# DJjjjhao/FIRA-ICSE

Measured on AMD Instinct MI355X. Metric: training commits/sec (FIRA default config), higher is better.
Workload: dtype f32; 1 GPU; BASELINE configs[1]: FIRA training step (fwd+bwd+Adam, dropout 0.1/0.2), batch 32 commits/GPU, fp32, 650-node graphs (mean nnz 1066/graph), vocab 24650; global_batch=32, parallelism=dp1

## Files before the change

### fira_icse_amd/_lib.py

```python
from __future__ import annotations

import ctypes as C
import os

HERE = os.path.dirname(os.path.abspath(__file__))
LIB_PATH = os.environ.get("FIRA_HIP_LIB") or os.path.join(HERE, "libfira_hip.so")


class FiraError(RuntimeError):
    pass


class Dims(C.Structure):
    _fields_ = [("sou_len", C.c_int32), ("sub_len", C.c_int32), ("ast_len", C.c_int32), ("tar_len", C.c_int32),
                ("d_model", C.c_int32), ("n_head", C.c_int32), ("n_layer", C.c_int32), ("vocab", C.c_int32),
                ("ast_vocab", C.c_int32), ("d_ff", C.c_int32)]


class Batch(C.Structure):
    _fields_ = [("B", C.c_int32), ("nnz", C.c_int32), ("sou", C.c_void_p), ("tar", C.c_void_p), ("mark", C.c_void_p),
                ("ast_change", C.c_void_p), ("tar_label", C.c_void_p), ("sub_token", C.c_void_p),
                ("n_nodes", C.c_int32), ("node_rows", C.c_void_p), ("rowptr", C.c_void_p), ("col", C.c_void_p),
                ("val", C.c_void_p), ("n_code", C.c_int32), ("code_rows", C.c_void_p), ("code_mark", C.c_void_p),
                ("n_mem", C.c_int32), ("mem_rows", C.c_void_p), ("mem_dst", C.c_void_p), ("head_rows", C.c_void_p),
# ... 36 lines not shown
    "fira_abi_version": (_I, []),
    "fira_param_count": (_I, [_DP]),
    "fira_param_info": (_I, [_DP, _I, C.c_char_p, C.POINTER(_L), C.POINTER(_L), C.POINTER(C.c_int32), C.POINTER(_L)]),
    "fira_param_total": (_L, [_DP]),
    "fira_workspace_bytes": (_Z, [_DP, _I, _I]),
    "fira_decode_workspace_bytes": (_Z, [_DP, _I, _I]),
    "fira_decode_workspace_bytes_ex": (_Z, [_DP, _I, _I, _I]),
    "fira_gemm_f32": (_I, [_P, _I, _I, _I, _I, _I, _P, _I, _P, _I, _P, _I, _P, _I, _I]),
    "fira_gemm_bf16": (_I, [_P, _I, _I, _I, _I, _I, _P, _I, _P, _I, _P, _I, _P, _I, _I]),
    "fira_weight_shadow": (_I, [_P, _I, _I, _P, _P, _P]),
    "fira_gemm_bf16_wb": (_I, [_P, _I, _I, _I, _P, _I, _P, _I, _P, _I, _P, _I, _I]),
    "fira_csr_spmm_f32": (_I, [_P, _I, _P, _P, _P, _P, _I, _P, _I, _I, _I]),
    "fira_csr_spmm": (_I, [_P, _I, _L, _P, _P, _P, _P, _I, _P, _I, _I, _I, _I]),
    "fira_gcn_layer_fwd": (_I, [_P, _I, _P, _P, _P, _P, _P, _P, _P, _P, _P, _P, _P, _P, _P, _F, _U64, _U32, _I]),
    "fira_gcn_layer_bwd": (_I, [_P, _I, _P, _P, _P, _P, _P, _P, _P, _I]),
    "fira_gcn_weight_planes": (_I, [_P, _I, _P, _P]),
    "fira_linear_x3": (_I, [_P, _I, _I, _P, _I, _P, _P, _P, _I, _I]),
    "fira_linear_dgrad_x3": (_I, [_P, _I, _I, _P, _I, _P, _P, _I, _I, _I]),
    "fira_dgrad_x3_splitk_planes_bytes": (_Z, [_I]),
    "fira_dgrad_x3_splitk": (_I, [_P, _I, _I, _P, _I, _P, _P, _P, _I, _I]),
    "fira_head_logits_x3_scratch_bytes": (_Z, [_I]),
    "fira_head_logits_x3": (_I, [_P, _I, _I, _P, _I, _P, _P, _P, _I, _P]),
    "fira_combination_block_fwd": (_I, [_P, _I, _P, _P, _P, _P, _P, _P, _P, _I, _P, _P, _P, _P, _P, _P, _P, _P, _P, _F, _U64, _U32, _U32, _I]),
    "fira_combination_block_bwd": (_I, [_P, _I, _P, _P, _P, _P, _P, _P, _P, _P, _P, _I, _P, _P, _P, _P, _P, _P, _I, _P, _F, _U64, _U32, _U32, _I]),
    "fira_combination_block_bwd_part_floats": (_I, []),
    "fira_embed_gather_fwd": (_I, [_P, _I, _I, _P, _P, _P, _P, _I, _I]),
    "fira_embed_gather_bwd": (_I, [_P, _I, _I, _P, _P, _P, _I, _I, _I]),
    "fira_combination_fwd": (_I, [_P, _I, _P, _P, _P, _P, _F, _U64, _U32]),
    "fira_combination_bwd": (_I, [_P, _I, _P, _P, _P, _P, _P, _P, _F, _U64, _U32]),
    "fira_add_layernorm_fwd": (_I, [_P, _I, _P, _P, _P, _P, _P, _P, _F, _U64, _U32]),
    "fira_linear_presum_f32": (_I, [_P, _I, _I, _P, _I, _P, _P, _P, _P, _F, _U64, _U32]),
    "fira_ln_linear_f32": (_I, [_P, _I, _I, _P, _I, _P, _P, _P, _I, _I, _P, _P, _P, _P]),
    "fira_ln_bwd_linear_f32": (_I, [_P, _I, _I, _P, _P, _P, _P, _P, _P, _P, _P, _P, _P, _P, _P, _F, _U64, _U32]),
    "fira_linear_layernorm_bf16_fwd": (_I, [_P, _I, _P, _I, _P, _I, _P, _P, _P, _P, _P, _P, _P, _F, _U64, _U32]),
    "fira_add_layernorm_bwd": (_I, [_P, _I, _P, _P, _P, _P, _P, _P, _P, _P, _F, _U64, _U32]),
    "fira_dropout_mask": (_I, [_P, _U64, _U32, _L, _F, _P]),
    "fira_colsum_f32": (_I, [_P, _I, _I, _P, _I, _P]),
    "fira_attention_fwd": (_I, [_P, _I, _I, _I, _I, _P, _I, _P, _I, _P, _I, _P, _I, _I, _P, _I]),
    "fira_attention_bwd": (_I, [_P, _I, _I, _I, _I, _P, _I, _P, _I, _P, _I, _P, _I, _I, _P, _I, _P, _I,
                                _P, _I, _P, _I, _P, _I]),
    "fira_attention_fwd_ex": (_I, [_P, _I, _I, _I, _I, _P, _I, _P, _I, _P, _I, _P, _I, _I, _P, _I, _P, _I, _I, _P]),
    "fira_attention_bwd_ex": (_I, [_P, _I, _I, _I, _I, _P, _I, _P, _I, _P, _I, _P, _I, _I, _P, _I, _P, _I,
                                   _P, _I, _P, _I, _P, _I, _P, _I, _I, _P]),
    "fira_decode_attention": (_I, [_P, _I, _I, _I, _P, _I, _P, _I, _P, _I, _P, _P, _I, _I, _I, _I, _P, _P, _I, _P, _P, _P]),
    "fira_copy_score_fwd": (_I, [_P, _I, _I, _I, _P, _P, _P, _P, _P]),
    "fira_copy_score_bwd": (_I, [_P, _I, _I, _I, _P, _P, _P, _P, _P, _P, _P, _P]),
    "fira_head_loss": (_I, [_P, _I, _I, _I, _I, _P, _P, _I, _P, _P, _P, _P, _P, _P, _P, _I]),
    "fira_adam_step": (_I, [_P, _L, _P, _P, _P, _P, _F, _F, _F, _F, _I, _P]),
    "fira_adam_step_mb": (_I, [_P, _L, _P, _P, _P, _P, _P, _F, _F, _F, _F, _I, _P, _P]),
    "fira_inv_count": (_I, [_P, _P, _P]),
    "fira_adam_step_count": (_I, [_P, _L, _P, _P, _P, _P, _F, _F, _F, _F, _I, _P]),
    "fira_pack_stats": (_I, [_P, _P, _P, _P]),
    "fira_debug_chain": (_I, [_P, _I, _I, _P]),
    "fira_train_fwd_bwd": (_I, [_P, _DP, _BP, _P, _P, _P, _Z, _OP, _P, _P, _P]),
    "fira_train_step": (_I, [_P, _DP, _BP, _P, _P, _P, _Z, _OP, _P, _P, C.POINTER(AdamOpts)]),
    "fira_gemm_wgrad_panel": (_I, [_P, _I, _I, _I, _I, _P, _I, _P, _I, _P, _I, _P, _P, _Z]),
    "fira_ffn_fwd": (_I, [_P, _I, _I] + [_P] * 11 + [_F, _U64, _U32, _I]),
    "fira_ffn_bwd": (_I, [_P, _I, _I] + [_P] * 17 + [_F, _U64, _U32, _I]),
    "fira_head_topk": (_I, [_P, _I, _I, _I, _P, _P, _P, _P, _I, _P, _P, _I]),
    "fira_train_step_rows": (_I, [_P, _DP, _BP, _P, _P, _P, _Z, _OP, _P, _P, C.POINTER(AdamOpts), _P]),
    "fira_adam_rows_sync": (_I, [_P, _DP, _P, C.POINTER(AdamOpts), _P]),
    "fira_adam_rows_catchup": (_I, [_P, _DP, _P, C.POINTER(AdamOpts), _P, _I, _P, _I]),
    "fira_adam_rows_step": (_I, [_P, _DP, _P, _P, C.POINTER(AdamOpts), _P, _P, _P, _I]),
    "fira_train_step_begin_rows": (_I, [_P, _DP, _BP, _P, _P, _P, _Z, _OP, _P, _P, _P, C.POINTER(AdamOpts), _P]),
    "fira_train_step_end_rows": (_I, [_P, _P, C.POINTER(AdamOpts), _P, _P, _P]),
    "fira_ema_update": (_I, [_P, _L, _P, _P, _F]),
# ... 120 lines not shown
```

### fira_icse_amd/csrc/gemm_small.hip

```cpp
#include "engine.h"
#include "epilogue.h"
#include <stdlib.h>

namespace fira {

typedef float f32x16 __attribute__((ext_vector_type(16)));
typedef float f32x4 __attribute__((ext_vector_type(4)));

template <bool B_KCONTIG>
__global__ __launch_bounds__(256) void gemm_small_kernel(int M, int N, int K, const float* __restrict__ A, int lda,
                                                         const float* __restrict__ B, int ldb, float* __restrict__ C,
                                                         int ldc, const float* __restrict__ bias, int flags,
                                                         const int32_t* __restrict__ c_rows,
                                                         const float* __restrict__ relu_mask) {
    __shared__ float red[4][1024];
    const int lane = threadIdx.x & 63, wave = threadIdx.x >> 6;
    const int l31 = lane & 31, kh = lane >> 5;
    const int m0 = blockIdx.y * 32, n0 = blockIdx.x * 32;
    const float* pa = A + (size_t)min(m0 + l31, M - 1) * lda + kh * 16;
    const float* pb = B_KCONTIG ? B + (size_t)min(n0 + l31, N - 1) * ldb + kh * 16
                                : B + (size_t)(kh * 16) * ldb + min(n0 + l31, N - 1);
    f32x16 acc;
#pragma unroll
    for (int r = 0; r < 16; ++r) acc[r] = 0.f;
// ... 105 lines not shown
        const char* pb = slot + 4096 + fb;
        f32x4 vb0, vb1, vb2, vb3;
        vb0.x = *reinterpret_cast<const float*>(pb);        vb0.y = *reinterpret_cast<const float*>(pb + 128);
        vb0.z = *reinterpret_cast<const float*>(pb + 256);  vb0.w = *reinterpret_cast<const float*>(pb + 384);
        vb1.x = *reinterpret_cast<const float*>(pb + 512);  vb1.y = *reinterpret_cast<const float*>(pb + 640);
        vb1.z = *reinterpret_cast<const float*>(pb + 768);  vb1.w = *reinterpret_cast<const float*>(pb + 896);
        vb2.x = *reinterpret_cast<const float*>(pb + 1024); vb2.y = *reinterpret_cast<const float*>(pb + 1152);
        vb2.z = *reinterpret_cast<const float*>(pb + 1280); vb2.w = *reinterpret_cast<const float*>(pb + 1408);
        vb3.x = *reinterpret_cast<const float*>(pb + 1536); vb3.y = *reinterpret_cast<const float*>(pb + 1664);
        vb3.z = *reinterpret_cast<const float*>(pb + 1792); vb3.w = *reinterpret_cast<const float*>(pb + 1920);
        FIRA_MFMA4(va0, vb0) FIRA_MFMA4(va1, vb1) FIRA_MFMA4(va2, vb2) FIRA_MFMA4(va3, vb3)
    }
    return acc;
}

struct LnA {
    const float* gamma = nullptr;
    const float* beta = nullptr;
    float* x_out = nullptr;
    float* stats_out = nullptr;
};

struct LnB {
    const float* sum = nullptr;
    const float* stats = nullptr;
    const float* gamma = nullptr;
    float* ds = nullptr;
    float* dx = nullptr;
    float* part = nullptr;
    float p = 0.f, inv_keep = 1.f;
    uint64_t seed = 0;
    uint32_t site = 0;
    uint32_t idx0 = 0;
};

template <bool B_KCONTIG, int NCH, bool LN_A = false, bool LN_B = false, int NW = 4>
__global__ __launch_bounds__(NW * 64) void gemm_tile32_kernel(int M, int N, const float* __restrict__ A, int lda,
                                                          const float* __restrict__ B, int ldb, float* __restrict__ C,
                                                          int ldc, const float* __restrict__ bias, int flags,
                                                          const int32_t* __restrict__ c_rows,
                                                          const float* __restrict__ relu_mask,
                                                          const int32_t* __restrict__ a_rows, int tiles_n, const EpiRes er,
                                                          const LnA ln, const LnB lb) {
    static_assert(NW == 4 || (!LN_A && !LN_B), "the LayerNorm prologues are written for four waves");
    extern __shared__ __attribute__((aligned(16))) char tile32_dyn[];
    __shared__ __attribute__((aligned(16))) char smem4[NW == 4 ? 4 * 8192 : 16];
    char* const smem = NW == 4 ? smem4 : tile32_dyn;
    __shared__ float ln_red[2][4][32];
    const int lane = threadIdx.x & 63;
    const int wave = __builtin_amdgcn_readfirstlane(threadIdx.x >> 6);
    int t;
    {
        const int b = blockIdx.x, nwg = gridDim.x, q = nwg >> 3, r = nwg & 7, x = b & 7;
        t = (x < r ? x * (q + 1) : r * (q + 1) + (x - r) * q) + (b >> 3);
    }
    const int m0 = (t / tiles_n) * 32, n0 = (t % tiles_n) * 32;
    char* slot = smem + wave * 8192;
    const int lr = lane >> 3, ls = lane & 7;
    const int sw_even = lr >> 1, sw_odd = 4 + (lr >> 1);
    int ra0 = min(m0 + lr, M - 1), ra1 = min(m0 + 8 + lr, M - 1), ra2 = min(m0 + 16 + lr, M - 1), ra3 = min(m0 + 24 + lr, M - 1);
    if (a_rows) { ra0 = a_rows[ra0]; ra1 = a_rows[ra1]; ra2 = a_rows[ra2]; ra3 = a_rows[ra3]; }
    const float* pa0 = A + (size_t)ra0 * lda + ((ls ^ sw_even) << 2);
    const float* pa1 = A + (size_t)ra1 * lda + ((ls ^ sw_odd) << 2);
    const float* pa2 = A + (size_t)ra2 * lda + ((ls ^ sw_even) << 2);
    const float* pa3 = A + (size_t)ra3 * lda + ((ls ^ sw_odd) << 2);
    const float *pb0, *pb1, *pb2, *pb3;
    if (B_KCONTIG) {
        pb0 = B + (size_t)min(n0 + lr, N - 1) * ldb + ((ls ^ sw_even) << 2);
        pb1 = B + (size_t)min(n0 + 8 + lr, N - 1) * ldb + ((ls ^ sw_odd) << 2);
        pb2 = B + (size_t)min(n0 + 16 + lr, N - 1) * ldb + ((ls ^ sw_even) << 2);
        pb3 = B + (size_t)min(n0 + 24 + lr, N - 1) * ldb + ((ls ^ sw_odd) << 2);
    } else {
        pb0 = B + (size_t)lr * ldb + n0 + (ls << 2);
        pb1 = pb0 + (size_t)8 * ldb;
        pb2 = pb0 + (size_t)16 * ldb;
        pb3 = pb0 + (size_t)24 * ldb;
    }
    const int i31 = lane & 31, kh = lane >> 5;
    const int wr_off = lr * 128 + ls * 16;
    const int sw_i = swz8(i31);
    const int fa0 = i31 * 128 + (((kh * 4 + 0) ^ sw_i) << 4), fa1 = i31 * 128 + (((kh * 4 + 1) ^ sw_i) << 4);
    const int fa2 = i31 * 128 + (((kh * 4 + 2) ^ sw_i) << 4), fa3 = i31 * 128 + (((kh * 4 + 3) ^ sw_i) << 4);
    const int fb = kh * 16 * 128 + i31 * 4;
    f32x16 acc;
#pragma unroll
    for (int r = 0; r < 16; ++r) acc[r] = 0.f;
    ChunkRegs R0, R1;
    tile32_fetch<B_KCONTIG>(R0, pa0, pa1, pa2, pa3, pb0, pb1, pb2, pb3, wave << 5, ldb);
    if (NCH > 1) tile32_fetch<B_KCONTIG>(R1, pa0, pa1, pa2, pa3, pb0, pb1, pb2, pb3, (wave + NW) << 5, ldb);
// ... 49 lines not shown
                if (r3 < M) { ln.stats_out[2 * r3] = mean[3]; ln.stats_out[2 * r3 + 1] = rstd[3]; }
            }
        }
    }
    if constexpr (LN_B) {
        static_assert(!LN_B || (NCH == 2 && !LN_A), "the LayerNorm-backward prologue needs the whole row in the two chunks of the four waves");
        auto hsum = [](const f32x4 v) { return (v.x + v.y) + (v.z + v.w); };
        const int ce = (ls ^ sw_even) << 2, co = (ls ^ sw_odd) << 2;
        const int k0 = wave << 5, k1 = (wave + 4) << 5;
        const float* ps0 = lb.sum + (size_t)ra0 * FIRA_D; const float* ps1 = lb.sum + (size_t)ra1 * FIRA_D;
        const float* ps2 = lb.sum + (size_t)ra2 * FIRA_D; const float* ps3 = lb.sum + (size_t)ra3 * FIRA_D;
        f32x4 s00 = *reinterpret_cast<const f32x4*>(ps0 + k0 + ce), s10 = *reinterpret_cast<const f32x4*>(ps0 + k1 + ce);
        f32x4 s01 = *reinterpret_cast<const f32x4*>(ps1 + k0 + co), s11 = *reinterpret_cast<const f32x4*>(ps1 + k1 + co);
        f32x4 s02 = *reinterpret_cast<const f32x4*>(ps2 + k0 + ce), s12 = *reinterpret_cast<const f32x4*>(ps2 + k1 + ce);
        f32x4 s03 = *reinterpret_cast<const f32x4*>(ps3 + k0 + co), s13 = *reinterpret_cast<const f32x4*>(ps3 + k1 + co);
        const float mean0 = lb.stats[2 * ra0], rstd0 = lb.stats[2 * ra0 + 1], mean1 = lb.stats[2 * ra1], rstd1 = lb.stats[2 * ra1 + 1];
        const float mean2 = lb.stats[2 * ra2], rstd2 = lb.stats[2 * ra2 + 1], mean3 = lb.stats[2 * ra3], rstd3 = lb.stats[2 * ra3 + 1];
        const f32x4 g0e = *reinterpret_cast<const f32x4*>(lb.gamma + k0 + ce), g0o = *reinterpret_cast<const f32x4*>(lb.gamma + k0 + co);
        const f32x4 g1e = *reinterpret_cast<const f32x4*>(lb.gamma + k1 + ce), g1o = *reinterpret_cast<const f32x4*>(lb.gamma + k1 + co);
        s00 = (s00 - mean0) * rstd0; s10 = (s10 - mean0) * rstd0; s01 = (s01 - mean1) * rstd1; s11 = (s11 - mean1) * rstd1;
        s02 = (s02 - mean2) * rstd2; s12 = (s12 - mean2) * rstd2; s03 = (s03 - mean3) * rstd3; s13 = (s13 - mean3) * rstd3;
        const f32x4 h00 = R0.a0 * g0e, h10 = R1.a0 * g1e, h01 = R0.a1 * g0o, h11 = R1.a1 * g1o;
        const f32x4 h02 = R0.a2 * g0e, h12 = R1.a2 * g1e, h03 = R0.a3 * g0o, h13 = R1.a3 * g1o;
        {
            const float p0 = sum8(hsum(h00) + hsum(h10)), p1 = sum8(hsum(h01) + hsum(h11));
            const float p2 = sum8(hsum(h02) + hsum(h12)), p3 = sum8(hsum(h03) + hsum(h13));
            const float q0 = sum8(hsum(h00 * s00) + hsum(h10 * s10)), q1 = sum8(hsum(h01 * s01) + hsum(h11 * s11));
            const float q2 = sum8(hsum(h02 * s02) + hsum(h12 * s12)), q3 = sum8(hsum(h03 * s03) + hsum(h13 * s13));
            if (ls == 0) {
                ln_red[0][wave][lr] = p0; ln_red[0][wave][8 + lr] = p1; ln_red[0][wave][16 + lr] = p2; ln_red[0][wave][24 + lr] = p3;
                ln_red[1][wave][lr] = q0; ln_red[1][wave][8 + lr] = q1; ln_red[1][wave][16 + lr] = q2; ln_red[1][wave][24 + lr] = q3;
            }
        }
        if (lb.part && n0 == 0) {
            const bool v0 = m0 + lr < M, v1 = m0 + 8 + lr < M, v2 = m0 + 16 + lr < M, v3 = m0 + 24 + lr < M;
            const f32x4 z = {0.f, 0.f, 0.f, 0.f};
            const f32x4 d00 = v0 ? R0.a0 : z, d10 = v0 ? R1.a0 : z, d01 = v1 ? R0.a1 : z, d11 = v1 ? R1.a1 : z;
            const f32x4 d02 = v2 ? R0.a2 : z, d12 = v2 ? R1.a2 : z, d03 = v3 ? R0.a3 : z, d13 = v3 ? R1.a3 : z;
            float* sc = reinterpret_cast<float*>(slot);
            float colsum[2];
#pragma unroll
            for (int pass = 0; pass < 2; ++pass) {
                __builtin_amdgcn_wave_barrier();
                *reinterpret_cast<f32x4*>(sc + (lr) * 64 + ce) = pass ? d00 : d00 * s00;
                *reinterpret_cast<f32x4*>(sc + (lr) * 64 + 32 + ce) = pass ? d10 : d10 * s10;
                *reinterpret_cast<f32x4*>(sc + (8 + lr) * 64 + co) = pass ? d01 : d01 * s01;
                *reinterpret_cast<f32x4*>(sc + (8 + lr) * 64 + 32 + co) = pass ? d11 : d11 * s11;
                *reinterpret_cast<f32x4*>(sc + (16 + lr) * 64 + ce) = pass ? d02 : d02 * s02;
                *reinterpret_cast<f32x4*>(sc + (16 + lr) * 64 + 32 + ce) = pass ? d12 : d12 * s12;
                *reinterpret_cast<f32x4*>(sc + (24 + lr) * 64 + co) = pass ? d03 : d03 * s03;
                *reinterpret_cast<f32x4*>(sc + (24 + lr) * 64 + 32 + co) = pass ? d13 : d13 * s13;
                __builtin_amdgcn_fence(__ATOMIC_RELEASE, "wavefront");
                __builtin_amdgcn_wave_barrier();
                __builtin_amdgcn_fence(__ATOMIC_ACQUIRE, "wavefront");
                float a0 = 0.f, a1 = 0.f;
#pragma unroll
                for (int r = 0; r < 32; r += 2) { a0 += sc[r * 64 + lane]; a1 += sc[(r + 1) * 64 + lane]; }
                colsum[pass] = a0 + a1;
            }
            const int col = ((wave + 4 * (lane >> 5)) << 5) + (lane & 31);
            float* pp = lb.part + (size_t)(m0 >> 5) * (2 * FIRA_D);
            pp[col] = colsum[0];
            pp[FIRA_D + col] = colsum[1];
        }
        __syncthreads();
        float m1[4], m2[4];
#pragma unroll
        for (int j = 0; j < 4; ++j) {
            m1[j] = ((ln_red[0][0][8 * j + lr] + ln_red[0][1][8 * j + lr]) + (ln_red[0][2][8 * j + lr] + ln_red[0][3][8 * j + lr])) * (1.0f / FIRA_D);
            m2[j] = ((ln_red[1][0][8 * j + lr] + ln_red[1][1][8 * j + lr]) + (ln_red[1][2][8 * j + lr] + ln_red[1][3][8 * j + lr])) * (1.0f / FIRA_D);
        }
        const f32x4 e00 = (h00 - m1[0] - s00 * m2[0]) * rstd0, e10 = (h10 - m1[0] - s10 * m2[0]) * rstd0;
        const f32x4 e01 = (h01 - m1[1] - s01 * m2[1]) * rstd1, e11 = (h11 - m1[1] - s11 * m2[1]) * rstd1;
        const f32x4 e02 = (h02 - m1[2] - s02 * m2[2]) * rstd2, e12 = (h12 - m1[2] - s12 * m2[2]) * rstd2;
        const f32x4 e03 = (h03 - m1[3] - s03 * m2[3]) * rstd3, e13 = (h13 - m1[3] - s13 * m2[3]) * rstd3;
        auto drop = [&](const f32x4 v, int row, int col) {
            if (lb.p <= 0.f) return v;
            const uint32_t e0 = lb.idx0 + (uint32_t)row * FIRA_D + (uint32_t)col;
            return f32x4{v.x * dropout_scale(lb.seed, lb.site, e0, lb.p, lb.inv_keep), v.y * dropout_scale(lb.seed, lb.site, e0 + 1, lb.p, lb.inv_keep),
                         v.z * dropout_scale(lb.seed, lb.site, e0 + 2, lb.p, lb.inv_keep), v.w * dropout_scale(lb.seed, lb.site, e0 + 3, lb.p, lb.inv_keep)};
        };
        const int r0 = m0 + lr, r1 = m0 + 8 + lr, r2 = m0 + 16 + lr, r3 = m0 + 24 + lr;
        R0.a0 = drop(e00, r0, k0 + ce); R1.a0 = drop(e10, r0, k1 + ce); R0.a1 = drop(e01, r1, k0 + co); R1.a1 = drop(e11, r1, k1 + co);
        R0.a2 = drop(e02, r2, k0 + ce); R1.a2 = drop(e12, r2, k1 + ce); R0.a3 = drop(e03, r3, k0 + co); R1.a3 = drop(e13, r3, k1 + co);
        if (n0 == 0) {
            float* o1 = lb.ds;
            float* o2 = lb.dx;
            if (r0 < M) { *reinterpret_cast<f32x4*>(o1 + (size_t)r0 * FIRA_D + k0 + ce) = e00; *reinterpret_cast<f32x4*>(o1 + (size_t)r0 * FIRA_D + k1 + ce) = e10;
                          *reinterpret_cast<f32x4*>(o2 + (size_t)r0 * FIRA_D + k0 + ce) = R0.a0; *reinterpret_cast<f32x4*>(o2 + (size_t)r0 * FIRA_D + k1 + ce) = R1.a0; }
            if (r1 < M) { *reinterpret_cast<f32x4*>(o1 + (size_t)r1 * FIRA_D + k0 + co) = e01; *reinterpret_cast<f32x4*>(o1 + (size_t)r1 * FIRA_D + k1 + co) = e11;
                          *reinterpret_cast<f32x4*>(o2 + (size_t)r1 * FIRA_D + k0 + co) = R0.a1; *reinterpret_cast<f32x4*>(o2 + (size_t)r1 * FIRA_D + k1 + co) = R1.a1; }
            if (r2 < M) { *reinterpret_cast<f32x4*>(o1 + (size_t)r2 * FIRA_D + k0 + ce) = e02; *reinterpret_cast<f32x4*>(o1 + (size_t)r2 * FIRA_D + k1 + ce) = e12;
                          *reinterpret_cast<f32x4*>(o2 + (size_t)r2 * FIRA_D + k0 + ce) = R0.a2; *reinterpret_cast<f32x4*>(o2 + (size_t)r2 * FIRA_D + k1 + ce) = R1.a2; }
            if (r3 < M) { *reinterpret_cast<f32x4*>(o1 + (size_t)r3 * FIRA_D + k0 + co) = e03; *reinterpret_cast<f32x4*>(o1 + (size_t)r3 * FIRA_D + k1 + co) = e13;
                          *reinterpret_cast<f32x4*>(o2 + (size_t)r3 * FIRA_D + k0 + co) = R0.a3; *reinterpret_cast<f32x4*>(o2 + (size_t)r3 * FIRA_D + k1 + co) = R1.a3; }
        }
    }
#pragma unroll
    for (int ci = 0; ci < NCH; ++ci) {
        if ((ci & 1) == 0) {
            tile32_stage(R0, slot, wr_off);
            if (ci + 2 < NCH) tile32_fetch<B_KCONTIG>(R0, pa0, pa1, pa2, pa3, pb0, pb1, pb2, pb3, (wave + NW * (ci + 2)) << 5, ldb);
        } else {
            tile32_stage(R1, slot, wr_off);
            if (ci + 2 < NCH) tile32_fetch<B_KCONTIG>(R1, pa0, pa1, pa2, pa3, pb0, pb1, pb2, pb3, (wave + NW * (ci + 2)) << 5, ldb);
        }
        acc = tile32_compute<B_KCONTIG>(slot, fa0, fa1, fa2, fa3, fb, acc);
    }
    __builtin_amdgcn_wave_barrier();
    float* red = reinterpret_cast<float*>(slot);
#pragma unroll
    for (int r = 0; r < 16; ++r) red[r * 64 + lane] = acc[r];
    __syncthreads();
    {
        constexpr int NV = (16 + NW - 1) / NW;
        const int lnn = threadIdx.x & 63;
        float vals[NV];
        int rows[NV];
        const float* p0 = reinterpret_cast<const float*>(smem);
#pragma unroll
        for (int i = 0; i < NV; ++i) {
            const int idx = threadIdx.x + NW * 64 * i, r = idx >> 6;
            const bool in = (16 % NW == 0) || idx < 1024;
            const int ix = in ? idx : threadIdx.x;
            if constexpr (NW == 4) {
                vals[i] = (p0[ix] + p0[2048 + ix]) + (p0[4096 + ix] + p0[6144 + ix]);
            } else {
                float v = 0.f;
#pragma unroll
                for (int w = 0; w < NW; w += 4)
// ... 72 lines not shown
            *rc = tile32_launch_wide(s, nw, K, tB, grid, M, N, A, lda, B, ldb, C, ldc, bias, flags, c_rows, relu_mask, a_rows, tiles_n, er);
            return true;
        }
    }
#define FIRA_T32(NCH)                                                                                                  \
    case NCH:                                                                                                          \
        if (tB) tile32_launch<true, NCH>(s, grid, M, N, A, lda, B, ldb, C, ldc, bias, flags, c_rows, relu_mask, a_rows, tiles_n, er); \
        else tile32_launch<false, NCH>(s, grid, M, N, A, lda, B, ldb, C, ldc, bias, flags, c_rows, relu_mask, a_rows, tiles_n, er); \
        break;
    switch (nch) { FIRA_T32(1) FIRA_T32(2) FIRA_T32(3) FIRA_T32(4) FIRA_T32(6) FIRA_T32(8) }
#undef FIRA_T32
    hipError_t e = hipGetLastError();
    *rc = e != hipSuccess ? set_err("gemm_tile32: %s", hipGetErrorString(e)) : 0;
    return true;
}

bool gemm_tile32_ln_try(hipStream_t s, int M, int N, const float* S, int lds, const float* W, const float* bias, float* Y,
                        int ldy, int flags, const float* gamma, const float* beta, float* x_out, float* stats_out, int* rc) {
    if (!gemm_tile32_takes(1, M, N, FIRA_D, S, lds, W, FIRA_D)) return false;
    if (((uintptr_t)gamma % 16) || ((uintptr_t)beta % 16) || ((uintptr_t)x_out % 16)) return false;
    ProfScope prof(s, PROF_GEMM, 2.0 * M * N * (double)FIRA_D, 4.0 * ((double)M * FIRA_D + (double)N * FIRA_D + (double)M * N));
    const int tiles_n = cdiv(N, 32);
    LnA ln;
    ln.gamma = gamma; ln.beta = beta; ln.x_out = x_out; ln.stats_out = stats_out;
    hipLaunchKernelGGL((gemm_tile32_kernel<true, 2, true, false>), dim3(cdiv(M, 32) * tiles_n), dim3(256), 0, s, M, N, S, lds, W, FIRA_D,
                       Y, ldy, bias, flags & 3, (const int32_t*)nullptr, (const float*)nullptr, (const int32_t*)nullptr, tiles_n,
                       EpiRes(), ln, LnB());
    hipError_t e = hipGetLastError();
    *rc = e != hipSuccess ? set_err("gemm_tile32_ln: %s", hipGetErrorString(e)) : 0;
    return true;
}

int gemm_tile32_lnb_blocks(int M) { return cdiv(M, 32); }
bool gemm_tile32_lnb_try(hipStream_t s, int M, int N, const float* dy, const float* W, int ldw, float* dX, int lddx,
                         const float* relu_mask, const float* sum, const float* stats, const float* gamma, float* ds,
                         float* dx_drop, float* part, float dropout, uint64_t seed, uint32_t site, int* rc, uint32_t idx0) {
    if (!gemm_tile32_takes(0, M, N, FIRA_D, dy, FIRA_D, W, ldw)) return false;
    if (((uintptr_t)sum % 16) || ((uintptr_t)gamma % 16) || ((uintptr_t)ds % 16) || ((uintptr_t)dx_drop % 16) || ds == dy) return false;
    ProfScope prof(s, PROF_GEMM, 2.0 * M * N * (double)FIRA_D, 4.0 * ((double)M * FIRA_D + (double)N * FIRA_D + (double)M * N));
    const int tiles_n = cdiv(N, 32);
    LnB lb;
    lb.sum = sum; lb.stats = stats; lb.gamma = gamma; lb.ds = ds; lb.dx = dx_drop; lb.part = part;
    lb.p = dropout; lb.inv_keep = dropout > 0.f ? 1.0f / (1.0f - dropout) : 1.0f; lb.seed = seed; lb.site = site; lb.idx0 = idx0;
    hipLaunchKernelGGL((gemm_tile32_kernel<false, 2, false, true>), dim3(cdiv(M, 32) * tiles_n), dim3(256), 0, s, M, N, dy, FIRA_D, W, ldw,
                       dX, lddx, (const float*)nullptr, 0, (const int32_t*)nullptr, relu_mask, (const int32_t*)nullptr, tiles_n,
                       EpiRes(), LnA(), lb);
    hipError_t e = hipGetLastError();
    *rc = e != hipSuccess ? set_err("gemm_tile32_lnb: %s", hipGetErrorString(e)) : 0;
    return true;
}

struct UnfoldGemm { const float *A, *B; float* C; int a_rs, a_ks, b_rs, b_ks, mode; };
struct UnfoldGemmTable { int n = 0; UnfoldGemm e[32]; };
__global__ __launch_bounds__(256) void unfold_gemm_kernel(const UnfoldGemmTable tab) {
    __shared__ float red[4][1024];
    const UnfoldGemm& q = tab.e[blockIdx.y];
    const int lane = threadIdx.x & 63, wave = threadIdx.x >> 6;
    const int l31 = lane & 31, kh = lane >> 5;
    if (q.mode == 2) {
        if (blockIdx.x >= 8) return;
        const f32x4 x = *reinterpret_cast<const f32x4*>(q.B + lane * 4);
        f32x4 a[8];
#pragma unroll
        for (int r = 0; r < 8; ++r)
            a[r] = *reinterpret_cast<const f32x4*>(q.A + (size_t)(blockIdx.x * 32 + wave * 8 + r) * q.a_rs + lane * 4);
#pragma unroll
        for (int r = 0; r < 8; ++r) {
            const float d = wave_sum((a[r].x * x.x + a[r].y * x.y) + (a[r].z * x.z + a[r].w * x.w));
            if (lane == 0) q.C[blockIdx.x * 32 + wave * 8 + r] = d;
        }
        return;
    }
    const int m0 = (blockIdx.x >> 3) * 32, n0 = (blockIdx.x & 7) * 32;
    const float* pa = q.A + (size_t)(m0 + l31) * q.a_rs;
    const float* pb = q.B + (size_t)(n0 + l31) * q.b_rs;
    f32x16 acc;
#pragma unroll
    for (int r = 0; r < 16; ++r) acc[r] = 0.f;
// ... 80 lines not shown
    constexpr long max_tiles = 1024;
    const long tiles = (long)cdiv(M, 32) * cdiv(N, 32);
    if (tA || (M > 64 && tiles > max_tiles) || K % 32 != 0 || K < 64 || lda % 4 != 0 || ((uintptr_t)A % 16) != 0) return false;
    if (tB && (ldb % 4 != 0 || ((uintptr_t)B % 16) != 0)) return false;
    if (gemm_tile32_try(s, tB, M, N, K, A, lda, B, ldb, C, ldc, bias, flags, rc, c_rows, relu_mask, nullptr, nullptr))
        return true;
    dim3 grid(cdiv(N, 32), cdiv(M, 32));
    if (tB) hipLaunchKernelGGL(gemm_small_kernel<true>, grid, dim3(256), 0, s, M, N, K, A, lda, B, ldb, C, ldc, bias, flags, c_rows, relu_mask);
    else hipLaunchKernelGGL(gemm_small_kernel<false>, grid, dim3(256), 0, s, M, N, K, A, lda, B, ldb, C, ldc, bias, flags, c_rows, relu_mask);
    hipError_t e = hipGetLastError();
    if (e != hipSuccess) *rc = set_err("gemm_small: %s", hipGetErrorString(e));
    return true;
}

}

extern "C" {
int fira_linear_presum_f32(void* stream, int M, int K, const float* X, int ldx, const float* W, const float* bias,
                           const float* res, float* sum, float dropout, uint64_t seed, uint32_t stream_id) {
    FIRA_REQUIRE(X && W && res && sum && M > 0, "fira_linear_presum_f32: bad argument");
    FIRA_REQUIRE(dropout >= 0.f && dropout < 1.f, "fira_linear_presum_f32: dropout must be in [0,1)");
    fira::EpiRes er;
    er.res = res; er.ldr = FIRA_D; er.p = dropout; er.inv_keep = dropout > 0.f ? 1.0f / (1.0f - dropout) : 1.0f;
    er.seed = seed; er.site = stream_id;
    int rc = 0;
    if (!fira::gemm_tile32_try((hipStream_t)stream, 1, M, FIRA_D, K, X, ldx, W, K, sum, FIRA_D, bias, 0, &rc, nullptr, nullptr,
                               nullptr, &er))
        return fira::set_err("fira_linear_presum_f32: shape %d x 256 x %d / alignment not taken by the tile kernel", M, K);
    return rc;
}
int fira_ln_bwd_linear_f32(void* stream, int M, int N, const float* dy, const float* Wt, float* dX, const float* relu_mask,
                           const float* sum, const float* stats, const float* gamma, float* ds, float* dx_drop, float* dgamma,
                           float* dbeta, float* part, float dropout, uint64_t seed, uint32_t site) {
    FIRA_REQUIRE(dy && Wt && dX && sum && stats && gamma && ds && dx_drop && dgamma && dbeta && part && M > 0 && N > 0,
                 "fira_ln_bwd_linear_f32: bad argument");
    FIRA_REQUIRE(ds != dy, "fira_ln_bwd_linear_f32: ds must not alias dy");
    FIRA_REQUIRE(dropout >= 0.f && dropout < 1.f, "fira_ln_bwd_linear_f32: dropout must be in [0,1)");
    int rc = 0;
    if (!fira::gemm_tile32_lnb_try((hipStream_t)stream, M, N, dy, Wt, N, dX, N, relu_mask, sum, stats, gamma, ds, dx_drop, part,
                                   dropout, seed, site, &rc))
        return fira::set_err("fira_ln_bwd_linear_f32: shape %d x %d / alignment not taken by the tile kernel", M, N);
    if (rc) return rc;
    fira::RedTable tab;
    const int nb = fira::gemm_tile32_lnb_blocks(M);
    tab.e[0] = fira::RedEntry{dgamma, part, FIRA_D, nb, 2 * FIRA_D};
    tab.e[1] = fira::RedEntry{dbeta, part + FIRA_D, FIRA_D, nb, 2 * FIRA_D};
    tab.n = 2;
    return fira::deferred_reduce((hipStream_t)stream, tab);
}
int fira_ln_linear_f32(void* stream, int M, int N, const float* S, int lds, const float* W, const float* bias, float* Y,
                       int ldy, int relu, const float* gamma, const float* beta, float* x_out, float* stats_out) {
    FIRA_REQUIRE(S && W && Y && gamma && beta && x_out && M > 0 && N > 0, "fira_ln_linear_f32: bad argument");
    int rc = 0;
    if (!fira::gemm_tile32_ln_try((hipStream_t)stream, M, N, S, lds, W, bias, Y, ldy, relu ? FIRA_GEMM_RELU : 0, gamma, beta, x_out,
                                  stats_out, &rc))
        return fira::set_err("fira_ln_linear_f32: shape %d x %d / alignment not taken by the tile kernel", M, N);
    return rc;
}
}
```

### fira_icse_amd/ops.py

```python
from __future__ import annotations

import dataclasses

import torch

from . import _lib
from ._lib import check, cur_stream, ptr


def _f32(t):
    assert t.is_cuda and t.dtype == torch.float32 and t.is_contiguous(), "expected a contiguous fp32 CUDA tensor"
    return t


def _i32(t):
    assert t.is_cuda and t.dtype == torch.int32 and t.is_contiguous(), "expected a contiguous int32 CUDA tensor"
    return t


def gemm(A, B, *, transA=False, transB=True, bias=None, relu=False, out=None, accumulate=False, splitk=1,
         tile=0, dtype="f32"):
    for t in (A, B):
        assert t.is_cuda and t.dtype == torch.float32 and t.dim() == 2 and t.stride(1) == 1
    M, K = (A.shape[1], A.shape[0]) if transA else A.shape
# ... 104 lines not shown
    assert w.shape[1] == 256 and s.shape[1] == 256 and s.stride(1) == 1
    y = torch.empty((M, N), dtype=torch.float32, device=s.device)
    x = torch.empty((M, 256), dtype=torch.float32, device=s.device)
    stats = torch.empty((M, 2), dtype=torch.float32, device=s.device)
    check(_lib.lib().fira_ln_linear_f32(cur_stream(), M, N, ptr(s), s.stride(0), ptr(_f32(w)), ptr(bias), ptr(y), N, int(relu),
                                        ptr(_f32(gamma)), ptr(_f32(beta)), ptr(x), ptr(stats)), "fira_ln_linear_f32")
    return y, x, stats


def linear_layernorm_bf16_fwd(x, wb, bias, res, gamma, beta, dropout=0.0, seed=0, site=0):
    M, K = x.shape
    assert K == 256 and wb.shape == (256, 256) and wb.dtype == torch.int16 and x.stride(1) == 1
    y = torch.empty((M, 256), dtype=torch.float32, device=x.device)
    s = torch.empty_like(y)
    stats = torch.empty((M, 2), dtype=torch.float32, device=x.device)
    check(_lib.lib().fira_linear_layernorm_bf16_fwd(cur_stream(), M, ptr(x), x.stride(0), ptr(wb), wb.stride(0), ptr(bias),
                                                    ptr(res), ptr(_f32(gamma)), ptr(_f32(beta)), ptr(s), ptr(y), ptr(stats),
                                                    dropout, seed, site), "fira_linear_layernorm_bf16_fwd")
    return y, s, stats


def add_layernorm_bwd(dy, s, stats, gamma, dropout=0.0, seed=0, site=0, want_dx_drop=False):
    M = dy.shape[0]
    ds = torch.empty_like(dy)
    dxd = torch.empty_like(dy) if want_dx_drop else None
    dg = torch.zeros(256, dtype=torch.float32, device=dy.device)
    db = torch.zeros(256, dtype=torch.float32, device=dy.device)
    check(_lib.lib().fira_add_layernorm_bwd(cur_stream(), M, ptr(_f32(dy)), ptr(_f32(s)), ptr(_f32(stats)),
                                            ptr(_f32(gamma)), ptr(ds), ptr(dxd), ptr(dg), ptr(db), dropout, seed, site),
          "fira_add_layernorm_bwd")
    return ds, dxd, dg, db


def ln_bwd_linear(dy, Wt, summ, stats, gamma, relu_mask=None, dropout=0.0, seed=0, site=0):
    M, N = dy.shape[0], Wt.shape[1]
    dX = torch.empty((M, N), dtype=torch.float32, device=dy.device)
    ds, dxd = torch.empty_like(dy), torch.empty_like(dy)
    dg = torch.zeros(256, dtype=torch.float32, device=dy.device)
    db = torch.zeros(256, dtype=torch.float32, device=dy.device)
    part = torch.empty(((M + 31) // 32) * 512, dtype=torch.float32, device=dy.device)
    check(_lib.lib().fira_ln_bwd_linear_f32(cur_stream(), M, N, ptr(_f32(dy)), ptr(_f32(Wt)), ptr(dX),
                                            ptr(None if relu_mask is None else _f32(relu_mask)), ptr(_f32(summ)),
                                            ptr(_f32(stats)), ptr(_f32(gamma)), ptr(ds), ptr(dxd), ptr(dg), ptr(db), ptr(part),
                                            dropout, seed, site), "fira_ln_bwd_linear_f32")
    return dX, ds, dxd, dg, db


def dropout_mask(seed, site, n, p, device="cuda"):
    out = torch.empty(n, dtype=torch.float32, device=device)
    check(_lib.lib().fira_dropout_mask(cur_stream(), seed, site, n, p, ptr(out)), "fira_dropout_mask")
    return out


def colsum(X):
    out = torch.zeros(X.shape[1], dtype=torch.float32, device=X.device)
    check(_lib.lib().fira_colsum_f32(cur_stream(), X.shape[0], X.shape[1], ptr(_f32(X)), X.stride(0), ptr(out)),
          "fira_colsum_f32")
    return out


def gcn_weight_planes(B):
    B = _f32(B).contiguous()
    n = B.numel() // (256 * 256)
    planes = torch.empty(n * 3 * 256 * 256, dtype=torch.int16, device=B.device)
    check(_lib.lib().fira_gcn_weight_planes(cur_stream(), n, ptr(B), ptr(planes)), "fira_gcn_weight_planes")
    return planes


def linear_x3(x, W, bias=None, dtype=2, ldo=None):
    x = _f32(x)
    M, N = x.shape[0], W.shape[0]
    planes = gcn_weight_planes(W)
    ldo = N if ldo is None else ldo
    out = torch.zeros((M, ldo), dtype=torch.float32, device=x.device)
    check(_lib.lib().fira_linear_x3(cur_stream(), M, N, ptr(x), x.stride(0), ptr(planes), ptr(None if bias is None else _f32(bias)),
                                    ptr(out), ldo, dtype), "fira_linear_x3")
    return out[:, :N]
# ... 429 lines not shown
```

### include/fira_hip.h

```cpp
#ifndef FIRA_HIP_H
#define FIRA_HIP_H

#include <stddef.h>
#include <stdint.h>

#ifdef __cplusplus
extern "C" {
#endif

#define FIRA_ABI_VERSION 10

typedef struct fira_dims {
    int32_t sou_len;
    int32_t sub_len;
    int32_t ast_len;
    int32_t tar_len;
    int32_t d_model;
    int32_t n_head;
    int32_t n_layer;
    int32_t vocab;
    int32_t ast_vocab;
    int32_t d_ff;
} fira_dims;

// ... 101 lines not shown
                               const float* WoT, const float* bqk, const float* bo, const float* vtab, int ldv,
                               const int32_t* mark, float* qk, float* c, const float* gamma, const float* beta, float* sum,
                               float* y, const int32_t* y_rows, float* stats, float dropout, uint64_t seed,
                               uint32_t site_gate, uint32_t site_out, int dtype);

int fira_combination_block_bwd(void* stream, int n_rows, float* dG, const int32_t* rows, const float* sum, const float* stats,
                               const float* gamma, const float* Wo, const float* Wqk, const float* qk, const float* vtab,
                               int ldv, const int32_t* mark, float* dYc, float* dqk, float* dgamma, float* dbeta,
                               float* dvtab, int lddv, float* part, float dropout, uint64_t seed, uint32_t site_gate,
                               uint32_t site_out, int dtype);
int fira_combination_block_bwd_part_floats(void);

int fira_embed_gather_fwd(void* stream, int B, int L, const int32_t* idx, const float* table,
                          const float* pos, float* out, int out_bstride, int out_off);
int fira_embed_gather_bwd(void* stream, int B, int L, const int32_t* idx, float* dtable,
                          const float* dout, int out_bstride, int out_off, int padding_idx);

int fira_combination_fwd(void* stream, int M, const float* qk, const float* vtab, const int32_t* mark,
                         float* out, float dropout, uint64_t seed, uint32_t stream_id);
int fira_combination_bwd(void* stream, int M, const float* qk, const float* vtab, const int32_t* mark,
                         const float* dout, float* dqk, float* dvtab ,
                         float dropout, uint64_t seed, uint32_t stream_id);

int fira_add_layernorm_fwd(void* stream, int M, float* x, const float* res, const float* gamma,
                           const float* beta, float* y, float* stats, float dropout, uint64_t seed,
                           uint32_t stream_id);
int fira_linear_presum_f32(void* stream, int M, int K, const float* X, int ldx, const float* W, const float* bias,
                           const float* res, float* sum, float dropout, uint64_t seed, uint32_t stream_id);
int fira_ln_linear_f32(void* stream, int M, int N, const float* S, int lds, const float* W, const float* bias, float* Y,
                       int ldy, int relu, const float* gamma, const float* beta, float* x_out, float* stats_out);
int fira_ln_bwd_linear_f32(void* stream, int M, int N, const float* dy, const float* Wt, float* dX, const float* relu_mask,
                           const float* sum, const float* stats, const float* gamma, float* ds, float* dx_drop,
                           float* dgamma, float* dbeta, float* part, float dropout, uint64_t seed, uint32_t site);
int fira_linear_layernorm_bf16_fwd(void* stream, int M, const float* X, int ldx, const uint16_t* Wb, int ldb,
                                   const float* bias, const float* res, const float* gamma, const float* beta,
                                   float* sum, float* y, float* stats, float dropout, uint64_t seed,
                                   uint32_t stream_id);
int fira_add_layernorm_bwd(void* stream, int M, const float* dy, const float* sum, const float* stats,
                           const float* gamma, float* ds, float* dx_drop, float* dgamma, float* dbeta,
                           float dropout, uint64_t seed, uint32_t stream_id);

#define FIRA_SITE_GATE 0
#define FIRA_SITE_COMB_OUT 1
#define FIRA_SITE_GCN 2
#define FIRA_SITE_SELF 3
#define FIRA_SITE_CROSS 4
#define FIRA_SITE_FFN 5
#define FIRA_SITE(layer, kind) ((uint32_t)((layer) * 8 + (kind) + 1))
int fira_dropout_mask(void* stream, uint64_t seed, uint32_t site, int64_t n, float p, float* out);

int fira_colsum_f32(void* stream, int M, int N, const float* X, int ldx, float* out);

int fira_attention_fwd(void* stream, int B, int H, int Tq, int Tk, const float* Q, int ldq,
                       const float* K, int ldk, const float* V, int ldv, const int32_t* key_valid,
                       int causal, int q_pos0, float* O, int ldo);
int fira_attention_bwd(void* stream, int B, int H, int Tq, int Tk, const float* Q, int ldq,
                       const float* K, int ldk, const float* V, int ldv, const int32_t* key_valid,
                       int causal, int q_pos0, const float* O, int ldo, const float* dO, int lddo,
                       float* dQ, int lddq, float* dK, int lddk, float* dV, int lddv);
int fira_attention_fwd_ex(void* stream, int B, int H, int Tq, int Tk, const float* Q, int ldq,
                          const float* K, int ldk, const float* V, int ldv, const int32_t* key_valid,
                          int causal, int q_pos0, float* O, int ldo, const int32_t* q_off, int self_kv, int dtype,
                          const int32_t* k_off);
int fira_attention_bwd_ex(void* stream, int B, int H, int Tq, int Tk, const float* Q, int ldq,
                          const float* K, int ldk, const float* V, int ldv, const int32_t* key_valid,
                          int causal, int q_pos0, const float* O, int ldo, const float* dO, int lddo,
// ... 227 lines not shown
```

Baseline: 13680 commits/s.

## Let each LayerNorm-backward GEMM workgroup cover several output tiles and split dgamma partials

The fused LayerNorm-backward plus linear kernel now has each workgroup compute up to four 32-column output tiles, so the LN-backward prologue (dy, stats, ds and dropout recompute) is done once per row block instead of once per tile. Per-wave column partials for dgamma and dbeta are spread across tile groups, so the first group no longer does that reduction alone. A new entry point takes an index offset and optional preallocated outputs. In exchange the grid is smaller and shared memory doubles, which can cut occupancy, and the tiles-per-workgroup choice is tied to a minimum grid size.

```diff
diff --git a/fira_icse_amd/_lib.py b/fira_icse_amd/_lib.py
--- a/fira_icse_amd/_lib.py
+++ b/fira_icse_amd/_lib.py
@@ -92,6 +92,7 @@
     "fira_linear_presum_f32": (_I, [_P, _I, _I, _P, _I, _P, _P, _P, _P, _F, _U64, _U32]),
     "fira_ln_linear_f32": (_I, [_P, _I, _I, _P, _I, _P, _P, _P, _I, _I, _P, _P, _P, _P]),
     "fira_ln_bwd_linear_f32": (_I, [_P, _I, _I, _P, _P, _P, _P, _P, _P, _P, _P, _P, _P, _P, _P, _F, _U64, _U32]),
+    "fira_ln_bwd_linear_at_f32": (_I, [_P, _I, _I, _P, _P, _P, _P, _P, _P, _P, _P, _P, _P, _P, _P, _F, _U64, _U32, _U32]),
     "fira_linear_layernorm_bf16_fwd": (_I, [_P, _I, _P, _I, _P, _I, _P, _P, _P, _P, _P, _P, _P, _F, _U64, _U32]),
     "fira_add_layernorm_bwd": (_I, [_P, _I, _P, _P, _P, _P, _P, _P, _P, _P, _F, _U64, _U32]),
     "fira_dropout_mask": (_I, [_P, _U64, _U32, _L, _F, _P]),
diff --git a/fira_icse_amd/csrc/gemm_small.hip b/fira_icse_amd/csrc/gemm_small.hip
--- a/fira_icse_amd/csrc/gemm_small.hip
+++ b/fira_icse_amd/csrc/gemm_small.hip
@@ -161,6 +161,8 @@
     uint64_t seed = 0;
     uint32_t site = 0;
     uint32_t idx0 = 0;
+    int tpw = 1;
+    int tiles = 1;
 };
 
 template <bool B_KCONTIG, int NCH, bool LN_A = false, bool LN_B = false, int NW = 4>
@@ -173,7 +175,7 @@
                                                           const LnA ln, const LnB lb) {
     static_assert(NW == 4 || (!LN_A && !LN_B), "the LayerNorm prologues are written for four waves");
     extern __shared__ __attribute__((aligned(16))) char tile32_dyn[];
-    __shared__ __attribute__((aligned(16))) char smem4[NW == 4 ? 4 * 8192 : 16];
+    __shared__ __attribute__((aligned(16))) char smem4[NW == 4 ? (LN_B ? 8 : 4) * 8192 : 16];
     char* const smem = NW == 4 ? smem4 : tile32_dyn;
     __shared__ float ln_red[2][4][32];
     const int lane = threadIdx.x & 63;
@@ -183,7 +185,7 @@
         const int b = blockIdx.x, nwg = gridDim.x, q = nwg >> 3, r = nwg & 7, x = b & 7;
         t = (x < r ? x * (q + 1) : r * (q + 1) + (x - r) * q) + (b >> 3);
     }
-    const int m0 = (t / tiles_n) * 32, n0 = (t % tiles_n) * 32;
+    const int m0 = (t / tiles_n) * 32, n0 = (t % tiles_n) * 32 * (LN_B ? lb.tpw : 1);
     char* slot = smem + wave * 8192;
     const int lr = lane >> 3, ls = lane & 7;
     const int sw_even = lr >> 1, sw_odd = 4 + (lr >> 1);
@@ -299,36 +301,41 @@
                 ln_red[1][wave][lr] = q0; ln_red[1][wave][8 + lr] = q1; ln_red[1][wave][16 + lr] = q2; ln_red[1][wave][24 + lr] = q3;
             }
         }
-        if (lb.part && n0 == 0) {
+        if (lb.part) {
+            const int grp = t % tiles_n;
             const bool v0 = m0 + lr < M, v1 = m0 + 8 + lr < M, v2 = m0 + 16 + lr < M, v3 = m0 + 24 + lr < M;
             const f32x4 z = {0.f, 0.f, 0.f, 0.f};
-            const f32x4 d00 = v0 ? R0.a0 : z, d10 = v0 ? R1.a0 : z, d01 = v1 ? R0.a1 : z, d11 = v1 ? R1.a1 : z;
-            const f32x4 d02 = v2 ? R0.a2 : z, d12 = v2 ? R1.a2 : z, d03 = v3 ? R0.a3 : z, d13 = v3 ? R1.a3 : z;
             float* sc = reinterpret_cast<float*>(slot);
-            float colsum[2];
-#pragma unroll
-            for (int pass = 0; pass < 2; ++pass) {
-                __builtin_amdgcn_wave_barrier();
-                *reinterpret_cast<f32x4*>(sc + (lr) * 64 + ce) = pass ? d00 : d00 * s00;
-                *reinterpret_cast<f32x4*>(sc + (lr) * 64 + 32 + ce) = pass ? d10 : d10 * s10;
-                *reinterpret_cast<f32x4*>(sc + (8 + lr) * 64 + co) = pass ? d01 : d01 * s01;
-                *reinterpret_cast<f32x4*>(sc + (8 + lr) * 64 + 32 + co) = pass ? d11 : d11 * s11;
-                *reinterpret_cast<f32x4*>(sc + (16 + lr) * 64 + ce) = pass ? d02 : d02 * s02;
-                *reinterpret_cast<f32x4*>(sc + (16 + lr) * 64 + 32 + ce) = pass ? d12 : d12 * s12;
-                *reinterpret_cast<f32x4*>(sc + (24 + lr) * 64 + co) = pass ? d03 : d03 * s03;
-                *reinterpret_cast<f32x4*>(sc + (24 + lr) * 64 + 32 + co) = pass ? d13 : d13 * s13;
-                __builtin_amdgcn_fence(__ATOMIC_RELEASE, "wavefront");
-                __builtin_amdgcn_wave_barrier();
-                __builtin_amdgcn_fence(__ATOMIC_ACQUIRE, "wavefront");
-                float a0 = 0.f, a1 = 0.f;
-#pragma unroll
-                for (int r = 0; r < 32; r += 2) { a0 += sc[r * 64 + lane]; a1 += sc[(r + 1) * 64 + lane]; }
-                colsum[pass] = a0 + a1;
-            }
-            const int col = ((wave + 4 * (lane >> 5)) << 5) + (lane & 31);
             float* pp = lb.part + (size_t)(m0 >> 5) * (2 * FIRA_D);
-            pp[col] = colsum[0];
-            pp[FIRA_D + col] = colsum[1];
+#pragma unroll
+            for (int u = 0; u < 2; ++u) {
+                if ((wave + 4 * u) % tiles_n != grp) continue;
+                const f32x4 d0 = v0 ? (u ? R1.a0 : R0.a0) : z, d1 = v1 ? (u ? R1.a1 : R0.a1) : z;
+                const f32x4 d2 = v2 ? (u ? R1.a2 : R0.a2) : z, d3 = v3 ? (u ? R1.a3 : R0.a3) : z;
+                const f32x4 x0 = u ? s10 : s00, x1 = u ? s11 : s01, x2 = u ? s12 : s02, x3 = u ? s13 : s03;
+                float colsum[2];
+#pragma unroll
+                for (int pass = 0; pass < 2; ++pass) {
+                    __builtin_amdgcn_wave_barrier();
+                    *reinterpret_cast<f32x4*>(sc + (lr) * 32 + ce) = pass ? d0 : d0 * x0;
+                    *reinterpret_cast<f32x4*>(sc + (8 + lr) * 32 + co) = pass ? d1 : d1 * x1;
+                    *reinterpret_cast<f32x4*>(sc + (16 + lr) * 32 + ce) = pass ? d2 : d2 * x2;
+                    *reinterpret_cast<f32x4*>(sc + (24 + lr) * 32 + co) = pass ? d3 : d3 * x3;
+                    __builtin_amdgcn_fence(__ATOMIC_RELEASE, "wavefront");
+                    __builtin_amdgcn_wave_barrier();
+                    __builtin_amdgcn_fence(__ATOMIC_ACQUIRE, "wavefront");
+                    float a = 0.f;
+#pragma unroll
+                    for (int r = 0; r < 32; r += 2) a += sc[(r + kh) * 32 + i31];
+                    const float o = __shfl_xor(a, 32);
+                    colsum[pass] = kh ? o + a : a + o;
+                }
+                if (kh == 0) {
+                    const int col = ((wave + 4 * u) << 5) + i31;
+                    pp[col] = colsum[0];
+                    pp[FIRA_D + col] = colsum[1];
+                }
+            }
         }
         __syncthreads();
         float m1[4], m2[4];
@@ -363,6 +370,54 @@
                           *reinterpret_cast<f32x4*>(o2 + (size_t)r3 * FIRA_D + k0 + co) = R0.a3; *reinterpret_cast<f32x4*>(o2 + (size_t)r3 * FIRA_D + k1 + co) = R1.a3; }
         }
     }
+    if constexpr (LN_B) {
+        static_assert(!LN_B || !B_KCONTIG, "the LayerNorm-backward product reads W as stored [256, N]");
+        const int ntile = min(lb.tpw, lb.tiles - (t % tiles_n) * lb.tpw);
+        const int lnn = threadIdx.x & 63;
+        const rsrc_t rC = buf_rsrc(C, 0x7fffffffu);
+        const rsrc_t rM = buf_rsrc(relu_mask ? (const void*)relu_mask : (const void*)C, relu_mask ? 0x7fffffffu : 0u);
+        unsigned orow[4];
+#pragma unroll
+        for (int i = 0; i < 4; ++i) {
+            const int r = (threadIdx.x + 256 * i) >> 6, row = m0 + (r & 3) + 8 * (r >> 2) + 4 * (lnn >> 5);
+            orow[i] = row < M ? (unsigned)row * (unsigned)ldc * 4u : FIRA_OOB;
+        }
+        for (int j = 0; j < ntile; ++j) {
+            const bool more = j + 1 < ntile;
+            const size_t nb = (size_t)(j + 1) * 32;
+            const unsigned cb = (unsigned)(n0 + j * 32 + (lnn & 31)) * 4u;
+            float keep[4];
+#pragma unroll
+            for (int i = 0; i < 4; ++i) keep[i] = buf_load_f32(rM, orow[i] == FIRA_OOB ? FIRA_OOB : orow[i] + cb);
+            asm volatile("" ::: "memory");
+            tile32_stage(R0, slot, wr_off);
+            if (more) {
+                const size_t ob = (size_t)(wave << 5) * ldb + nb;
+                R0.b0 = *reinterpret_cast<const f32x4*>(pb0 + ob); R0.b1 = *reinterpret_cast<const f32x4*>(pb1 + ob);
+                R0.b2 = *reinterpret_cast<const f32x4*>(pb2 + ob); R0.b3 = *reinterpret_cast<const f32x4*>(pb3 + ob);
+            }
+            acc = tile32_compute<B_KCONTIG>(slot, fa0, fa1, fa2, fa3, fb, acc);
+            tile32_stage(R1, slot, wr_off);
+            if (more) {
+                const size_t ob = (size_t)((wave + 4) << 5) * ldb + nb;
+                R1.b0 = *reinterpret_cast<const f32x4*>(pb0 + ob); R1.b1 = *reinterpret_cast<const f32x4*>(pb1 + ob);
+                R1.b2 = *reinterpret_cast<const f32x4*>(pb2 + ob); R1.b3 = *reinterpret_cast<const f32x4*>(pb3 + ob);
+            }
+            acc = tile32_compute<B_KCONTIG>(slot, fa0, fa1, fa2, fa3, fb, acc);
+            float* redj = reinterpret_cast<float*>(smem + 4 * 8192) + (j & 1) * 4096;
+#pragma unroll
+            for (int r = 0; r < 16; ++r) { redj[wave * 1024 + r * 64 + lane] = acc[r]; acc[r] = 0.f; }
+            __syncthreads();
+#pragma unroll
+            for (int i = 0; i < 4; ++i) {
+                const int ix = threadIdx.x + 256 * i;
+                float v = (redj[ix] + redj[1024 + ix]) + (redj[2048 + ix] + redj[3072 + ix]);
+                if (relu_mask) v = keep[i] > 0.f ? v : 0.f;
+                __builtin_amdgcn_raw_buffer_store_b32(__builtin_bit_cast(unsigned, v), rC, orow[i] == FIRA_OOB ? FIRA_OOB : orow[i] + cb, 0, 0);
+            }
+        }
+        return;
+    }
 #pragma unroll
     for (int ci = 0; ci < NCH; ++ci) {
         if ((ci & 1) == 0) {
@@ -501,18 +556,27 @@
 }
 
 int gemm_tile32_lnb_blocks(int M) { return cdiv(M, 32); }
+static int lnb_tiles_per_wg(int M, int N) {
+    constexpr int LNB_MIN_GRID = 128;
+    const int rb = cdiv(M, 32), tn = cdiv(N, 32);
+    if (rb * cdiv(tn, 4) >= LNB_MIN_GRID) return 4;
+    if (rb * cdiv(tn, 2) >= LNB_MIN_GRID) return 2;
+    return 1;
+}
 bool gemm_tile32_lnb_try(hipStream_t s, int M, int N, const float* dy, const float* W, int ldw, float* dX, int lddx,
                          const float* relu_mask, const float* sum, const float* stats, const float* gamma, float* ds,
                          float* dx_drop, float* part, float dropout, uint64_t seed, uint32_t site, int* rc, uint32_t idx0) {
-    if (!gemm_tile32_takes(0, M, N, FIRA_D, dy, FIRA_D, W, ldw)) return false;
+    if (!gemm_tile32_takes(0, M, N, FIRA_D, dy, FIRA_D, W, ldw) || !epilogue_fits(M, lddx)) return false;
     if (((uintptr_t)sum % 16) || ((uintptr_t)gamma % 16) || ((uintptr_t)ds % 16) || ((uintptr_t)dx_drop % 16) || ds == dy) return false;
     ProfScope prof(s, PROF_GEMM, 2.0 * M * N * (double)FIRA_D, 4.0 * ((double)M * FIRA_D + (double)N * FIRA_D + (double)M * N));
-    const int tiles_n = cdiv(N, 32);
     LnB lb;
+    lb.tiles = cdiv(N, 32);
+    lb.tpw = lnb_tiles_per_wg(M, N);
+    const int groups_n = cdiv(lb.tiles, lb.tpw);
     lb.sum = sum; lb.stats = stats; lb.gamma = gamma; lb.ds = ds; lb.dx = dx_drop; lb.part = part;
     lb.p = dropout; lb.inv_keep = dropout > 0.f ? 1.0f / (1.0f - dropout) : 1.0f; lb.seed = seed; lb.site = site; lb.idx0 = idx0;
-    hipLaunchKernelGGL((gemm_tile32_kernel<false, 2, false, true>), dim3(cdiv(M, 32) * tiles_n), dim3(256), 0, s, M, N, dy, FIRA_D, W, ldw,
-                       dX, lddx, (const float*)nullptr, 0, (const int32_t*)nullptr, relu_mask, (const int32_t*)nullptr, tiles_n,
+    hipLaunchKernelGGL((gemm_tile32_kernel<false, 2, false, true>), dim3(cdiv(M, 32) * groups_n), dim3(256), 0, s, M, N, dy, FIRA_D, W, ldw,
+                       dX, lddx, (const float*)nullptr, 0, (const int32_t*)nullptr, relu_mask, (const int32_t*)nullptr, groups_n,
                        EpiRes(), LnA(), lb);
     hipError_t e = hipGetLastError();
     *rc = e != hipSuccess ? set_err("gemm_tile32_lnb: %s", hipGetErrorString(e)) : 0;
@@ -659,13 +723,19 @@
 int fira_ln_bwd_linear_f32(void* stream, int M, int N, const float* dy, const float* Wt, float* dX, const float* relu_mask,
                            const float* sum, const float* stats, const float* gamma, float* ds, float* dx_drop, float* dgamma,
                            float* dbeta, float* part, float dropout, uint64_t seed, uint32_t site) {
+    return fira_ln_bwd_linear_at_f32(stream, M, N, dy, Wt, dX, relu_mask, sum, stats, gamma, ds, dx_drop, dgamma, dbeta, part, dropout,
+                                     seed, site, 0);
+}
+int fira_ln_bwd_linear_at_f32(void* stream, int M, int N, const float* dy, const float* Wt, float* dX, const float* relu_mask,
+                              const float* sum, const float* stats, const float* gamma, float* ds, float* dx_drop, float* dgamma,
+                              float* dbeta, float* part, float dropout, uint64_t seed, uint32_t site, uint32_t idx0) {
     FIRA_REQUIRE(dy && Wt && dX && sum && stats && gamma && ds && dx_drop && dgamma && dbeta && part && M > 0 && N > 0,
                  "fira_ln_bwd_linear_f32: bad argument");
     FIRA_REQUIRE(ds != dy, "fira_ln_bwd_linear_f32: ds must not alias dy");
     FIRA_REQUIRE(dropout >= 0.f && dropout < 1.f, "fira_ln_bwd_linear_f32: dropout must be in [0,1)");
     int rc = 0;
     if (!fira::gemm_tile32_lnb_try((hipStream_t)stream, M, N, dy, Wt, N, dX, N, relu_mask, sum, stats, gamma, ds, dx_drop, part,
-                                   dropout, seed, site, &rc))
+                                   dropout, seed, site, &rc, idx0))
         return fira::set_err("fira_ln_bwd_linear_f32: shape %d x %d / alignment not taken by the tile kernel", M, N);
     if (rc) return rc;
     fira::RedTable tab;
diff --git a/fira_icse_amd/ops.py b/fira_icse_amd/ops.py
--- a/fira_icse_amd/ops.py
+++ b/fira_icse_amd/ops.py
@@ -160,17 +160,22 @@
     return ds, dxd, dg, db
 
 
-def ln_bwd_linear(dy, Wt, summ, stats, gamma, relu_mask=None, dropout=0.0, seed=0, site=0):
+def ln_bwd_linear(dy, Wt, summ, stats, gamma, relu_mask=None, dropout=0.0, seed=0, site=0, idx0=0, out=None):
     M, N = dy.shape[0], Wt.shape[1]
-    dX = torch.empty((M, N), dtype=torch.float32, device=dy.device)
-    ds, dxd = torch.empty_like(dy), torch.empty_like(dy)
+    if out is None:
+        dX = torch.empty((M, N), dtype=torch.float32, device=dy.device)
+        ds, dxd = torch.empty_like(dy), torch.empty_like(dy)
+        part = torch.empty(((M + 31) // 32) * 512, dtype=torch.float32, device=dy.device)
+    else:
+        dX, ds, dxd, part = (_f32(t) for t in out)
+        assert dX.shape[1] == N and dX.shape[0] >= M and ds.shape[0] >= M and dxd.shape[0] >= M
+        assert part.numel() >= ((M + 31) // 32) * 512
     dg = torch.zeros(256, dtype=torch.float32, device=dy.device)
     db = torch.zeros(256, dtype=torch.float32, device=dy.device)
-    part = torch.empty(((M + 31) // 32) * 512, dtype=torch.float32, device=dy.device)
-    check(_lib.lib().fira_ln_bwd_linear_f32(cur_stream(), M, N, ptr(_f32(dy)), ptr(_f32(Wt)), ptr(dX),
-                                            ptr(None if relu_mask is None else _f32(relu_mask)), ptr(_f32(summ)),
-                                            ptr(_f32(stats)), ptr(_f32(gamma)), ptr(ds), ptr(dxd), ptr(dg), ptr(db), ptr(part),
-                                            dropout, seed, site), "fira_ln_bwd_linear_f32")
+    check(_lib.lib().fira_ln_bwd_linear_at_f32(cur_stream(), M, N, ptr(_f32(dy)), ptr(_f32(Wt)), ptr(dX),
+                                               ptr(None if relu_mask is None else _f32(relu_mask)), ptr(_f32(summ)),
+                                               ptr(_f32(stats)), ptr(_f32(gamma)), ptr(ds), ptr(dxd), ptr(dg), ptr(db), ptr(part),
+                                               dropout, seed, site, idx0), "fira_ln_bwd_linear_at_f32")
     return dX, ds, dxd, dg, db
 
 
diff --git a/include/fira_hip.h b/include/fira_hip.h
--- a/include/fira_hip.h
+++ b/include/fira_hip.h
@@ -157,6 +157,9 @@
 int fira_ln_bwd_linear_f32(void* stream, int M, int N, const float* dy, const float* Wt, float* dX, const float* relu_mask,
                            const float* sum, const float* stats, const float* gamma, float* ds, float* dx_drop,
                            float* dgamma, float* dbeta, float* part, float dropout, uint64_t seed, uint32_t site);
+int fira_ln_bwd_linear_at_f32(void* stream, int M, int N, const float* dy, const float* Wt, float* dX, const float* relu_mask,
+                              const float* sum, const float* stats, const float* gamma, float* ds, float* dx_drop,
+                              float* dgamma, float* dbeta, float* part, float dropout, uint64_t seed, uint32_t site, uint32_t idx0);
 int fira_linear_layernorm_bf16_fwd(void* stream, int M, const float* X, int ldx, const uint16_t* Wb, int ldb,
                                    const float* bias, const float* res, const float* gamma, const float* beta,
                                    float* sum, float* y, float* stats, float dropout, uint64_t seed,
```

Result: no change. 13740 commits/s, median of 4 (+0.4%).
